# andrewmilson/sandstorm

Hardware: AMD Instinct MI355X
Metric: prove_wall_time_s (lower is better)
Workload: dtype u256 (Fp252, Montgomery R=2^256, 8 x u32 limbs)

## Files before the change

include/sandstorm_hip.h:

```cpp
#ifndef SANDSTORM_HIP_H
#define SANDSTORM_HIP_H
#include <stddef.h>
#include <stdint.h>

#ifdef __cplusplus
extern "C" {
#endif

typedef int ss_status;
enum {
    SS_OK = 0,
    SS_ERR_INVALID = 1,
    SS_ERR_HIP = 2,
    SS_ERR_NO_DEVICE = 3,
    SS_ERR_UNSUPPORTED = 4
};

typedef struct ss_ctx ss_ctx;

enum { SS_NTT_FORWARD = 0, SS_NTT_INVERSE = 1 };
enum { SS_ORDER_NATURAL = 0, SS_ORDER_BITREV = 1 };

enum {
    SS_HASH_KECCAK = 0,
// ... 20 lines not shown
void ss_ctx_destroy(ss_ctx *ctx);
ss_status ss_ctx_set_stream(ss_ctx *ctx, void *hip_stream);
ss_status ss_ctx_sync(ss_ctx *ctx);
ss_status ss_dev_alloc(ss_ctx *ctx, size_t bytes, void **d_out);
ss_status ss_dev_free(ss_ctx *ctx, void *d_ptr);
ss_status ss_ctx_trim(ss_ctx *ctx);
ss_status ss_upload(ss_ctx *ctx, void *d_dst, const void *src, size_t bytes);
ss_status ss_download(ss_ctx *ctx, void *dst, const void *d_src, size_t bytes);
ss_status ss_upload_async(ss_ctx *ctx, void *d_dst, const void *src, size_t bytes, uint64_t *ticket);
ss_status ss_wait_upload(ss_ctx *ctx, uint64_t ticket);
ss_status ss_dev_zero(ss_ctx *ctx, void *d_ptr, size_t bytes);

ss_status ss_dev_copy(ss_ctx *ctx, void *d_dst, const void *d_src, size_t bytes);
ss_status ss_dev_copy_2d(ss_ctx *ctx, void *d_dst, size_t dst_pitch, const void *d_src, size_t src_pitch, size_t width, size_t rows);
ss_status ss_bitrev_permute32(ss_ctx *ctx, const void *d_src, uint32_t log_n, void *d_dst);

typedef struct ss_comm ss_comm;
ss_status ss_comm_unique_id(uint8_t id_out[128]);
ss_status ss_comm_create(ss_ctx *ctx, const uint8_t id[128], uint32_t rank, uint32_t world, ss_comm **out);
void ss_comm_destroy(ss_comm *comm);
ss_status ss_comm_exchange(ss_comm *comm, uint32_t nsend, const uint32_t *send_peer, const void *const *d_send, const uint64_t *send_bytes,
                           uint32_t nrecv, const uint32_t *recv_peer, void *const *d_recv, const uint64_t *recv_bytes);
ss_status ss_comm_all_gather(ss_comm *comm, const void *d_send, uint64_t bytes, void *d_recv);

ss_status ss_ntt_fp252(ss_ctx *ctx, uint64_t *const *d_cols, uint32_t ncols, uint32_t log_n,
                       int direction, const uint64_t offset[4], int in_order, int out_order);

ss_status ss_lde_fp252(ss_ctx *ctx, const uint64_t *const *d_in, uint32_t ncols, uint32_t log_n,
                       uint32_t log_blowup, const uint64_t offset[4], uint64_t *const *d_evals,
                       uint64_t *const *d_coeffs);

ss_status ss_evaluate_fp252(ss_ctx *ctx, const uint64_t *const *d_coeffs, uint32_t ncols, uint32_t log_n,
                            uint32_t log_blowup, const uint64_t offset[4], uint64_t *const *d_evals);

ss_status ss_subsample_rows(ss_ctx *ctx, const uint64_t *const *d_in, uint32_t ncols, uint64_t nrows_out, uint32_t log_stride,
                            uint64_t *const *d_out);

enum { SS_NTT_PART_LOCAL = 0, SS_NTT_PART_CROSS = 1 };
ss_status ss_ntt_shard_fp252(ss_ctx *ctx, uint64_t *const *d_cols, uint32_t ncols, uint32_t log_n, uint32_t log_ranks,
                             uint32_t rank, int direction, const uint64_t offset[4], int part, uint32_t log_expand,
                             uint64_t *const *d_out);

ss_status ss_hash_rows(ss_ctx *ctx, int hash_kind, const uint64_t *const *d_cols, uint32_t ncols,
                       uint64_t nrows, uint8_t *d_digests);
ss_status ss_hash_rows_ex(ss_ctx *ctx, int hash_kind, const uint64_t *const *d_cols, uint32_t ncols,
                       uint64_t nrows, int row_order, uint8_t *d_digests);

ss_status ss_merkle_build(ss_ctx *ctx, int tree_kind, uint32_t n_friendly_layers, int leaf_kind,
                          const void *d_leaves, uint64_t n, uint8_t *d_nodes, uint8_t *d_tags,
                          uint8_t root_out[33]);
ss_status ss_merkle_build_ex(ss_ctx *ctx, int tree_kind, uint32_t n_friendly_layers, int leaf_kind,
                          const void *d_leaves, uint64_t n, int leaf_order, uint8_t *d_nodes, uint8_t *d_tags,
                          uint8_t root_out[33]);
ss_status ss_merkle_open(ss_ctx *ctx, const uint8_t *d_nodes, const uint8_t *d_tags, uint64_t n,
                         const uint64_t *idx, uint32_t nidx, uint8_t *out, uint8_t *out_tags);
ss_status ss_gather_rows(ss_ctx *ctx, const uint64_t *const *d_cols, uint32_t ncols,
                         const uint64_t *idx, uint32_t nidx, uint64_t *out );
typedef struct ss_gather_job {
    const void *const *d_cols;
    uint32_t ncols;
    uint32_t entry_bytes;
    const uint64_t *idx;
    uint32_t nidx;
    void *out;
} ss_gather_job;
ss_status ss_gather_batch(ss_ctx *ctx, const ss_gather_job *jobs, uint32_t njobs);
// ... 267 lines not shown
```

sandstorm_amd/_lib.py:

```python
import ctypes as C
import os
import sys

_HERE = os.path.dirname(os.path.abspath(__file__))
LIB_PATH = os.path.join(_HERE, "_build", "libsandstorm_hip.so")

HEADER_PATH = os.path.join(os.path.dirname(_HERE), "include", "sandstorm_hip.h")

SS_OK = 0


def header_abi_version():
    import re
    with open(HEADER_PATH) as f:
        m = re.search(r"#define\s+SS_ABI_VERSION\s+(\d+)u?", f.read())
    if not m:
        raise SandstormHipError("SS_ABI_VERSION not found in %s" % HEADER_PATH)
    return int(m.group(1))


class SandstormHipError(RuntimeError):
    pass


# ... 28 lines not shown

SIGNATURES = {
    "ss_last_error": (C.c_char_p, []),
    "ss_abi_version": (C.c_uint32, []),
    "ss_ctx_create": (C.c_int, [C.c_int, _vpp]),
    "ss_ctx_destroy": (None, [C.c_void_p]),
    "ss_ctx_set_stream": (C.c_int, [C.c_void_p, C.c_void_p]),
    "ss_ctx_sync": (C.c_int, [C.c_void_p]),
    "ss_dev_alloc": (C.c_int, [C.c_void_p, C.c_size_t, _vpp]),
    "ss_dev_free": (C.c_int, [C.c_void_p, C.c_void_p]),
    "ss_ctx_trim": (C.c_int, [C.c_void_p]),
    "ss_upload": (C.c_int, [C.c_void_p, C.c_void_p, C.c_void_p, C.c_size_t]),
    "ss_download": (C.c_int, [C.c_void_p, C.c_void_p, C.c_void_p, C.c_size_t]),
    "ss_dev_zero": (C.c_int, [C.c_void_p, C.c_void_p, C.c_size_t]),
    "ss_dev_copy": (C.c_int, [C.c_void_p, C.c_void_p, C.c_void_p, C.c_size_t]),
    "ss_dev_copy_2d": (C.c_int, [C.c_void_p, C.c_void_p, C.c_size_t, C.c_void_p, C.c_size_t, C.c_size_t, C.c_size_t]),
    "ss_bitrev_permute32": (C.c_int, [C.c_void_p, C.c_void_p, C.c_uint32, C.c_void_p]),
    "ss_comm_unique_id": (C.c_int, [C.c_char_p]),
    "ss_comm_create": (C.c_int, [C.c_void_p, C.c_char_p, C.c_uint32, C.c_uint32, _vpp]),
    "ss_comm_destroy": (None, [C.c_void_p]),
    "ss_comm_exchange": (C.c_int, [C.c_void_p, C.c_uint32, _u32p, _vpp, _u64p, C.c_uint32, _u32p, _vpp, _u64p]),
    "ss_comm_all_gather": (C.c_int, [C.c_void_p, C.c_void_p, C.c_uint64, C.c_void_p]),
    "ss_permutation_product": (C.c_int, [C.c_void_p, C.POINTER(PermOperand), C.POINTER(PermOperand), C.c_uint64, _u64p, _u64p,
                                         C.c_void_p, C.c_uint64, C.c_uint64, _u64p]),
    "ss_diluted_aggregate": (C.c_int, [C.c_void_p, C.c_void_p, C.c_uint64, C.c_uint64, C.c_uint64, _u64p, _u64p,
                                       C.c_void_p, C.c_uint64, C.c_uint64]),
    "ss_scale_strided": (C.c_int, [C.c_void_p, C.c_void_p, C.c_uint64, C.c_uint64, C.c_uint64, _u64p]),
    "ss_diluted_aggregate_block": (C.c_int, [C.c_void_p, C.c_void_p, C.c_uint64, C.c_uint64, C.c_uint64, C.c_int, _u64p, _u64p,
                                             C.c_void_p, _u64p]),
    "ss_affine_apply": (C.c_int, [C.c_void_p, C.c_void_p, C.c_uint64, _u64p, C.c_void_p, C.c_uint64, C.c_uint64]),
    "ss_ntt_fp252": (C.c_int, [C.c_void_p, _vpp, C.c_uint32, C.c_uint32, C.c_int, _u64p, C.c_int, C.c_int]),
    "ss_lde_fp252": (C.c_int, [C.c_void_p, _vpp, C.c_uint32, C.c_uint32, C.c_uint32, _u64p, _vpp, _vpp]),
    "ss_evaluate_fp252": (C.c_int, [C.c_void_p, _vpp, C.c_uint32, C.c_uint32, C.c_uint32, _u64p, _vpp]),
    "ss_subsample_rows": (C.c_int, [C.c_void_p, _vpp, C.c_uint32, C.c_uint64, C.c_uint32, _vpp]),
    "ss_ntt_shard_fp252": (C.c_int, [C.c_void_p, _vpp, C.c_uint32, C.c_uint32, C.c_uint32, C.c_uint32, C.c_int, _u64p, C.c_int, C.c_uint32, _vpp]),
    "ss_hash_rows": (C.c_int, [C.c_void_p, C.c_int, _vpp, C.c_uint32, C.c_uint64, C.c_void_p]),
    "ss_hash_rows_ex": (C.c_int, [C.c_void_p, C.c_int, _vpp, C.c_uint32, C.c_uint64, C.c_int, C.c_void_p]),
    "ss_merkle_build": (C.c_int, [C.c_void_p, C.c_int, C.c_uint32, C.c_int, C.c_void_p, C.c_uint64,
                                  C.c_void_p, C.c_void_p, _u8p]),
    "ss_merkle_build_ex": (C.c_int, [C.c_void_p, C.c_int, C.c_uint32, C.c_int, C.c_void_p, C.c_uint64, C.c_int,
                                  C.c_void_p, C.c_void_p, _u8p]),
    "ss_merkle_open": (C.c_int, [C.c_void_p, C.c_void_p, C.c_void_p, C.c_uint64, _u64p, C.c_uint32,
                                 C.c_void_p, C.c_void_p]),
    "ss_gather_rows": (C.c_int, [C.c_void_p, _vpp, C.c_uint32, _u64p, C.c_uint32, C.c_void_p]),
    "ss_gather_batch": (C.c_int, [C.c_void_p, C.POINTER(GatherJob), C.c_uint32]),
    "ss_trace_memory_image": (C.c_int, [C.c_void_p, C.c_void_p, C.c_uint64, C.c_void_p, C.c_uint64]),
    "ss_trace_cpu_cells": (C.c_int, [C.c_void_p, C.c_void_p, C.c_void_p, C.c_uint64, C.c_void_p, C.c_uint64, _u64p, C.c_uint64, C.c_void_p, C.c_void_p,
                                     C.c_void_p, C.c_void_p, C.c_void_p, C.c_void_p]),
    "ss_trace_builtin": (C.c_int, [C.c_void_p, _vpp, C.c_uint32, C.c_void_p, C.c_uint32, C.c_void_p, C.c_uint32, C.c_void_p, C.c_uint64, C.c_uint64,
                                   C.c_uint64, C.c_uint64, C.c_void_p]),
    "ss_trace_pedersen": (C.c_int, [C.c_void_p, _vpp, C.c_uint32, C.c_uint64, C.c_void_p, C.c_void_p, C.c_uint64, C.c_uint64, C.c_uint64, C.c_uint64, C.c_void_p,
                                    C.c_void_p]),
    "ss_trace_bitwise": (C.c_int, [C.c_void_p, _vpp, C.c_uint32, C.c_uint64, C.c_void_p, C.c_void_p, C.c_uint64, C.c_uint64, C.c_uint64, C.c_uint64, C.c_uint32,
                                   C.c_void_p, C.c_void_p]),
    "ss_trace_poseidon": (C.c_int, [C.c_void_p, _vpp, C.c_uint32, C.c_uint64, C.c_void_p, C.c_void_p, C.c_void_p, C.c_uint64, C.c_uint64, C.c_uint64, C.c_uint64,
                                    C.c_void_p, C.c_void_p]),
    "ss_trace_ec_op": (C.c_int, [C.c_void_p, _vpp, C.c_uint32, C.c_uint64, C.c_void_p, C.c_void_p, C.c_uint64, C.c_uint64, C.c_uint64, C.c_uint64, C.c_void_p,
                                 C.c_void_p]),
    "ss_trace_ecdsa": (C.c_int, [C.c_void_p, _vpp, C.c_uint32, C.c_uint64, C.c_void_p, C.c_void_p, C.c_void_p, C.c_uint64, C.c_uint64, C.c_uint64, C.c_uint64,
                                 C.c_void_p, C.c_void_p]),
    "ss_trace_rc_pool": (C.c_int, [C.c_void_p, C.c_void_p, C.c_void_p, C.c_void_p, C.c_uint64, C.c_void_p]),
    "ss_trace_rc_builtin": (C.c_int, [C.c_void_p, C.c_void_p, C.c_void_p, C.c_void_p, C.c_void_p, C.c_void_p, C.c_void_p]),
    "ss_trace_ordered_runs": (C.c_int, [C.c_void_p, C.c_void_p, C.c_uint64, C.c_uint64, C.c_uint64, C.c_void_p, C.c_uint32, C.c_uint32, C.c_int]),
    "ss_trace_patch": (C.c_int, [C.c_void_p, C.c_void_p, C.c_uint64, C.c_void_p, C.c_void_p, C.c_uint64]),
    "ss_trace_ordered_memory": (C.c_int, [C.c_void_p, C.c_uint64, C.c_void_p, C.c_void_p, C.c_void_p, C.c_void_p, C.c_void_p, C.c_uint32, C.c_uint64, _u64p,
                                          C.c_uint32, C.c_void_p]),
# ... 83 lines not shown
```

sandstorm_amd/csrc/capi.hip:

```cpp
#include <hip/hip_runtime.h>
#include <dlfcn.h>
#include <algorithm>
#include <cstdarg>
#include <chrono>
#include <cstdio>
#include <cstdlib>
#include <cstring>
#include <map>
#include <mutex>
#include <string>
#include <tuple>
#include <utility>
#include <vector>

#include "../../include/sandstorm_hip.h"
#include "fp252.h"
#include "fp252_host.h"
#include "kernels.h"
#include "quotient_gen.h"
#include "ext_scan.h"
#include "gl_ntt.h"

using namespace ss;

// ... 356 lines not shown
            s0 += r; rem -= r;
        }
    }
    return v;
}

ss_status run_forward(ss_ctx *ctx, const ColPtrs &cols, uint32_t ncols, uint32_t log_n, const Fp *tw,
                      uint32_t log_expand, bool canonical_out = true) {
    const uint32_t lt = (uint32_t)ntt_log_tile_max();
    const uint32_t log_tile = log_n < lt ? log_n : lt;
    std::vector<Pass> passes = plan_passes(log_n);
    if (log_expand >= log_n && log_n > 0) return fail(SS_ERR_INVALID, "log_blowup %u too large", log_expand);
    size_t start = 0;
    uint32_t skip = log_expand;
    while (start + 1 < passes.size() && skip >= passes[start].r) { skip -= passes[start].r; ++start; }
    if (skip >= passes[start].r && log_n > 0) return fail(SS_ERR_INVALID, "log_blowup %u too large", log_expand);
    ColPtrs inplace = cols;
    for (uint32_t c = 0; c < ncols; ++c) inplace.src[c] = cols.dst[c];
    for (size_t i = start; i < passes.size(); ++i) {
        const bool first = i == start;
        ss_ctx::Scope prof(ctx, SS_PROF_NTT_PASS);
        HIP_TRY(launch_ntt_pass(ctx->stream, NTT_MODE_DIT, first ? cols : inplace, ncols, tw, log_n, passes[i].s0,
                                passes[i].r, log_tile, first ? skip : 0, first ? log_expand : 0, 0, canonical_out && i + 1 == passes.size()));
    }
    return SS_OK;
}
ss_status get_inverse_plan(ss_ctx *ctx, uint32_t log_n, const Fp &offset, const Fp **tw, int *mode) {
    static const bool force_dif = getenv("SS_NTT_INVERSE_DIF") != nullptr;
    const bool cti = fp_eq(offset, fp_one()) && !force_dif;
    *mode = cti ? NTT_MODE_CTI : NTT_MODE_DIF;
    return ctx->get_plan(log_n, true, offset, tw, cti);
}
ss_status run_inverse(ss_ctx *ctx, const ColPtrs &cols, uint32_t ncols, uint32_t log_n, const Fp *tw, int mode,
                      uint32_t scale_log = ~0u, bool cti_trivial = true) {
    if (scale_log == ~0u) scale_log = log_n;
    const uint32_t lt = (uint32_t)ntt_log_tile_max();
    const uint32_t log_tile = log_n < lt ? log_n : lt;
    std::vector<Pass> passes = plan_passes(log_n);
    ColPtrs inplace = cols;
    for (uint32_t c = 0; c < ncols; ++c) inplace.src[c] = cols.dst[c];
    for (size_t i = passes.size(); i-- > 0;) {
        const bool first = i == passes.size() - 1;
        const bool last = i == 0;
        ss_ctx::Scope prof(ctx, SS_PROF_NTT_PASS);
        HIP_TRY(launch_ntt_pass(ctx->stream, mode, first ? cols : inplace, ncols, tw, log_n, passes[i].s0,
                                passes[i].r, log_tile, 0, 0, last ? scale_log : 0, last, cti_trivial));
    }
    return SS_OK;
}

bool valid_log(uint32_t log_n) { return log_n >= 1 && log_n <= 30; }

}

extern "C" {

const char *ss_last_error(void) { return g_err.c_str(); }
uint32_t ss_abi_version(void) { return SS_ABI_VERSION; }

ss_status ss_ctx_create(int device, ss_ctx **out) {
    if (!out) return fail(SS_ERR_INVALID, "out is NULL");
    int count = 0;
    hipError_t e = hipGetDeviceCount(&count);
    if (e != hipSuccess || count <= 0)
        return fail(SS_ERR_NO_DEVICE, "no HIP device: %s", e == hipSuccess ? "device count is 0" : hipGetErrorString(e));
    if (device < 0 || device >= count) return fail(SS_ERR_INVALID, "device %d out of range (%d)", device, count);
    HIP_TRY(hipSetDevice(device));
    hipDeviceProp_t prop;
    HIP_TRY(hipGetDeviceProperties(&prop, device));
    if (strncmp(prop.gcnArchName, "gfx950", 6) != 0)
        return fail(SS_ERR_NO_DEVICE, "device %d is %s; this library is built for gfx950 only", device, prop.gcnArchName);
    ss_ctx *ctx = new ss_ctx;
    ctx->device = device;
    HIP_TRY(hipStreamCreateWithFlags(&ctx->own_stream, hipStreamNonBlocking));
    ctx->stream = ctx->own_stream;
    HIP_TRY(hipMalloc(&ctx->d_small, 64 * sizeof(uint64_t)));
    HIP_TRY(ntt_set_func_attributes());
    HIP_TRY(gl_set_func_attributes());
    *out = ctx;
// ... 396 lines not shown
        ColPtrs inv, fwd;
        memset(&inv, 0, sizeof inv); memset(&fwd, 0, sizeof fwd);
        for (uint32_t c = 0; c < nc; ++c) {
            void *co = d_coeffs ? (void *)d_coeffs[base + c] : (void *)((char *)ctx->scratch + col_bytes * c);
            inv.src[c] = d_in[base + c]; inv.dst[c] = co;
            fwd.src[c] = co; fwd.dst[c] = d_evals[base + c];
        }
        st = run_inverse(ctx, inv, nc, log_n, tw_inv, inv_mode);
        if (st != SS_OK) return st;
        st = run_forward(ctx, fwd, nc, log_n + log_blowup, tw_fwd, log_blowup);
        if (st != SS_OK) return st;
    }
    return SS_OK;
}

ss_status ss_evaluate_fp252(ss_ctx *ctx, const uint64_t *const *d_coeffs, uint32_t ncols, uint32_t log_n,
                            uint32_t log_blowup, const uint64_t offset[4], uint64_t *const *d_evals) {
    if (!ctx || !d_coeffs || !d_evals) return fail(SS_ERR_INVALID, "NULL argument");
    if (!valid_log(log_n) || !valid_log(log_n + log_blowup)) return fail(SS_ERR_INVALID, "size out of range");
    if (has_null((const void *const *)d_coeffs, ncols) || has_null((const void *const *)d_evals, ncols)) return fail(SS_ERR_INVALID, "NULL column");
    const Fp off = offset ? fp_from_limbs64(offset) : fp_one();
    const Fp *tw = nullptr;
    ss_status st = ctx->get_plan(log_n + log_blowup, false, off, &tw);
    if (st != SS_OK) return st;
    for (uint32_t base = 0; base < ncols; base += MAX_COLS) {
        const uint32_t nc = ncols - base < (uint32_t)MAX_COLS ? ncols - base : (uint32_t)MAX_COLS;
        ColPtrs fwd;
        memset(&fwd, 0, sizeof fwd);
        for (uint32_t c = 0; c < nc; ++c) { fwd.src[c] = d_coeffs[base + c]; fwd.dst[c] = d_evals[base + c]; }
        st = run_forward(ctx, fwd, nc, log_n + log_blowup, tw, log_blowup);
        if (st != SS_OK) return st;
    }
    return SS_OK;
}

ss_status ss_subsample_rows(ss_ctx *ctx, const uint64_t *const *d_in, uint32_t ncols, uint64_t nrows_out, uint32_t log_stride,
                            uint64_t *const *d_out) {
    if (!ctx || !d_in || !d_out) return fail(SS_ERR_INVALID, "NULL argument");
    if (!ncols || !nrows_out) return fail(SS_ERR_INVALID, "no columns or no rows");
    if (log_stride > 4) return fail(SS_ERR_INVALID, "log_stride %u > 4", log_stride);
    if (nrows_out > (1ull << 40)) return fail(SS_ERR_INVALID, "size out of range");
    if (has_null((const void *const *)d_in, ncols) || has_null((const void *const *)d_out, ncols)) return fail(SS_ERR_INVALID, "NULL column");
    for (uint32_t base = 0; base < ncols; base += MAX_COLS) {
        const uint32_t nc = ncols - base < (uint32_t)MAX_COLS ? ncols - base : (uint32_t)MAX_COLS;
        ColPtrs cols;
        memset(&cols, 0, sizeof cols);
        for (uint32_t c = 0; c < nc; ++c) { cols.src[c] = d_in[base + c]; cols.dst[c] = d_out[base + c]; }
        HIP_TRY(launch_subsample_rows(ctx->stream, cols, nc, nrows_out, log_stride));
    }
    return SS_OK;
}

ss_status ss_ntt_shard_fp252(ss_ctx *ctx, uint64_t *const *d_cols, uint32_t ncols, uint32_t log_n, uint32_t log_ranks, uint32_t rank,
                             int direction, const uint64_t offset[4], int part, uint32_t log_expand, uint64_t *const *d_out) {
    if (!ctx || !d_cols) return fail(SS_ERR_INVALID, "NULL argument");
    if (direction != SS_NTT_FORWARD && direction != SS_NTT_INVERSE) return fail(SS_ERR_INVALID, "bad direction");
    if (part != SS_NTT_PART_LOCAL && part != SS_NTT_PART_CROSS) return fail(SS_ERR_INVALID, "bad part");
    if (!valid_log(log_n) || log_ranks == 0 || 2 * log_ranks > log_n || log_ranks > 7) return fail(SS_ERR_INVALID, "a transform of 2^%u points does not split over 2^%u ranks (needs n >= R^2)", log_n, log_ranks);
    if (rank >> log_ranks) return fail(SS_ERR_INVALID, "rank %u of %u", rank, 1u << log_ranks);
    if (ncols == 0) return fail(SS_ERR_INVALID, "no columns");
    if (has_null((const void *const *)d_cols, ncols) || (d_out && has_null((const void *const *)d_out, ncols))) return fail(SS_ERR_INVALID, "NULL column");
    for (uint32_t c0 = 0; ncols > (uint32_t)MAX_COLS && c0 < ncols; c0 += MAX_COLS) {
        const uint32_t k = ncols - c0 < (uint32_t)MAX_COLS ? ncols - c0 : (uint32_t)MAX_COLS;
        const ss_status st = ss_ntt_shard_fp252(ctx, d_cols + c0, k, log_n, log_ranks, rank, direction, offset, part, log_expand, d_out ? d_out + c0 : nullptr);
        if (st != SS_OK || c0 + k == ncols) return st;
    }
// ... 2185 lines not shown
```

sandstorm_amd/csrc/kernels.h:

```cpp
#pragma once
#include <hip/hip_runtime.h>
#include <stdint.h>
#include "fp252.h"

namespace ss {

static constexpr int MAX_COLS = 16;

struct ColPtrs {
    const void *src[MAX_COLS];
    void *dst[MAX_COLS];
};
struct ConstColPtrs {
    const void *p[MAX_COLS];
};

int ntt_log_tile_max();
static constexpr size_t NTT_PLAN_ENTRY_BYTES = 36;
enum { NTT_MODE_DIT = 0, NTT_MODE_DIF = 1, NTT_MODE_CTI = 2 };
struct NttWindow { uint32_t first, log_len; };
hipError_t launch_ntt_pass(hipStream_t st, int mode, const ColPtrs &cols, uint32_t ncols, const Fp *tw,
                           uint32_t log_n, uint32_t s0, uint32_t r, uint32_t log_tile, uint32_t u_first,
                           uint32_t log_expand, uint32_t scale_pow2, bool final_pass, bool cti_trivial = true,
                           const NttWindow *win = nullptr, uint64_t tw_entries = 0);
hipError_t launch_twiddles(hipStream_t st, Fp *tw, const Fp *pow_lo, const Fp *pow_hi, const Fp *hpow,
                           uint32_t log_n, bool h_is_one, bool bitrev_levels, const NttWindow *win = nullptr, uint32_t win_stages = 0);
static inline uint64_t ntt_window_plan_entries(const NttWindow &win, uint32_t stages) { return (((uint64_t)1 << stages) - 1ull) << win.log_len; }
hipError_t launch_bitrev(hipStream_t st, Fp *a, uint32_t log_n);
hipError_t launch_mul_bench(hipStream_t st, const Fp *a, const Fp *b, Fp *out, uint64_t n, uint32_t reps);
hipError_t ntt_set_func_attributes();

hipError_t launch_hash_rows(hipStream_t st, int kind, const ConstColPtrs &cols, uint32_t ncols,
                            uint64_t nrows, uint32_t brev_bits, uint8_t *digests);
hipError_t launch_bitrev_copy(hipStream_t st, const Fp *src, uint32_t log_n, Fp *dst);
hipError_t launch_hash_pairs(hipStream_t st, int kind, const uint8_t *in, uint64_t count, uint8_t *out);
hipError_t launch_hash_felt_pairs(hipStream_t st, int kind, const Fp *felts, uint64_t count, bool bitrev, uint8_t *out, uint8_t *leaves);
hipError_t launch_felts_to_be(hipStream_t st, const Fp *felts, uint64_t count, uint8_t *out);
hipError_t launch_pow_prefix(hipStream_t st, int coin_kind, const uint8_t digest[32], uint32_t bits,
                             uint64_t *d_prefix);
hipError_t launch_pow_grind(hipStream_t st, int coin_kind, const uint64_t *d_prefix, uint32_t bits,
                            uint64_t start, uint64_t count, unsigned long long *d_best);
hipError_t launch_gather32(hipStream_t st, const uint8_t *in, const uint64_t *d_idx, uint64_t n, uint8_t *out);
hipError_t launch_gather32_cols(hipStream_t st, const void *const *d_cols, uint32_t ncols, uint32_t c0, uint32_t row_cols, const uint64_t *d_idx,
                                uint64_t nidx, uint8_t *out);
hipError_t launch_gather8(hipStream_t st, const uint8_t *in, const uint64_t *d_idx, uint64_t n, uint8_t *out);

struct PedersenTables;
hipError_t pedersen_tables_create(hipStream_t st, PedersenTables **out);
void pedersen_tables_destroy(PedersenTables *t);
void pedersen_tables_trim();
static constexpr uint64_t PEDERSEN_TMP_FELTS_PER_HASH = 4;
hipError_t launch_pedersen_felts(hipStream_t st, const PedersenTables *t, const Fp *a, const Fp *b,
                                 uint64_t n, Fp *out, Fp *tmp);
hipError_t launch_pedersen_pairs(hipStream_t st, const PedersenTables *t, const uint8_t *in, uint64_t count,
                                 uint8_t *out, Fp *tmp);
hipError_t launch_pedersen_felt_pairs(hipStream_t st, const PedersenTables *t, const Fp *felts,
                                      uint64_t count, uint8_t *out, Fp *tmp);
// ... 212 lines not shown
```

sandstorm_amd/csrc/ntt.hip:

```cpp
#include <hip/hip_runtime.h>
#include <cstdlib>
#include "fp252.h"
#include "fl252.h"
#include "kernels.h"

#ifdef SS_NTT_ABL_NOBAR
#define NTT_SYNC() do {} while (0)
#else
#define NTT_SYNC() __syncthreads()
#endif
#ifndef SS_NTT_WAVE_PRIVATE
#define SS_NTT_WAVE_PRIVATE 1
#endif
#if defined(HIPEMU)
#define NTT_WAVE_SYNC() __syncthreads()
#elif defined(SS_NTT_ABL_NOBAR)
#define NTT_WAVE_SYNC() do {} while (0)
#else
#define NTT_WAVE_SYNC() do { __builtin_amdgcn_fence(__ATOMIC_RELEASE, "wavefront"); __builtin_amdgcn_wave_barrier(); \
                             __builtin_amdgcn_fence(__ATOMIC_ACQUIRE, "wavefront"); } while (0)
#endif

namespace ss {

// ... 107 lines not shown
    const uint4 *q = reinterpret_cast<const uint4 *>(p);
    uint4 a = q[0], b = q[1];
    Fp r;
    r.v[0] = a.x; r.v[1] = a.y; r.v[2] = a.z; r.v[3] = a.w;
    r.v[4] = b.x; r.v[5] = b.y; r.v[6] = b.z; r.v[7] = b.w;
    return r;
}
__device__ __forceinline__ void gstore(Fp *p, const Fp &x) {
#ifdef SS_NTT_ABL_NOGL
    if (!(x.v[0] == 0xdeadbeefu && x.v[3] == 77u)) return;
#endif
    uint4 *q = reinterpret_cast<uint4 *>(p);
    q[0] = make_uint4(x.v[0], x.v[1], x.v[2], x.v[3]);
    q[1] = make_uint4(x.v[4], x.v[5], x.v[6], x.v[7]);
}

struct PassParams {
    uint32_t log_n;
    uint32_t s0;
    uint32_t r;
    uint32_t log_tile;
    uint32_t u_first;
    uint32_t log_expand;
    uint32_t scale_pow2;
    uint32_t contig;
    uint32_t final_pass;
    uint32_t ncols;
    uint32_t xcd_map;
    uint32_t log_tiles;
    uint32_t tile0;
    uint32_t win_log1, win0;
    uint32_t cti_trivial;
    uint32_t tw_entries;
};
__device__ __forceinline__ uint32_t mem_index(const PassParams &p, uint32_t g) {
    if (!p.win_log1) return g;
    return ((g >> p.s0) << (p.win_log1 - 1u)) + ((g & ((1u << p.s0) - 1u)) - p.win0);
}

struct TwPlanes {
    const uint4 *lo, *hi;
    const u32 *top;
};
__device__ __forceinline__ Fl tw_load(const TwPlanes &tw, uint32_t idx) {
    const uint4 a4 = tw.lo[idx], b4 = tw.hi[idx];
    Fl t;
    t.l[0] = a4.x; t.l[1] = a4.y; t.l[2] = a4.z; t.l[3] = a4.w;
    t.l[4] = b4.x; t.l[5] = b4.y; t.l[6] = b4.z; t.l[7] = b4.w;
    t.l[8] = tw.top[idx];
    return t;
}

template <int MODE, int G, int ST>
__device__ __forceinline__ uint32_t stage_tw_index(const PassParams &p, uint32_t u, uint32_t g0, int pr) {
    constexpr int STC = ST < G ? ST : 0;
    const uint32_t gsh = p.s0 + u;
    const uint32_t s = gsh + STC;
    if (MODE == MODE_CTI) {
        const uint32_t level = p.log_n - 1u - s;
        return ((1u << level) - 1u) + ((g0 >> (gsh + G)) << (G - 1 - STC)) + (uint32_t)(pr >> STC);
    }
    const uint32_t klow = g0 & ((1u << gsh) - 1u);
    const int m = ((pr >> STC) << (STC + 1)) | (pr & ((1 << STC) - 1));
    if (p.win_log1)
        return ((((1u << (s - p.s0)) - 1u) + (klow >> p.s0)) << (p.win_log1 - 1u)) + ((klow & ((1u << p.s0) - 1u)) - p.win0)
               + ((uint32_t)(m & ((1 << STC) - 1)) << (u + p.win_log1 - 1u));
// ... 230 lines not shown
    if (MODE == MODE_DIT) {
        uint32_t u = p.u_first;
        bool first = true;
        while (u < p.r) {
            const uint32_t g = (p.r - u) >= (uint32_t)NTT_GMAX ? (uint32_t)NTT_GMAX : (p.r - u);
            const bool last = (u + g >= p.r);
            const bool fg = fuse && first, tg = fuse && last;
            if (fg) prev_private = group_private(u, g); else phase_sync(group_private(u, g));
            if (NTT_GMAX >= 3 && g == 3) radix_group<MODE, NTT_GMAX >= 3 ? 3 : 1>(t, tw, p, u, tile, false, fg, tg, src, dst);
            else if (g == 2) radix_group<MODE, 2>(t, tw, p, u, tile, false, fg, tg, src, dst);
            else radix_group<MODE, 1>(t, tw, p, u, tile, false, fg, tg, src, dst);
            u += g;
            first = false;
        }
    } else {
        uint32_t u = p.r;
        bool first = true;
        const bool top_pass = p.s0 + p.r == p.log_n;
        while (u > 0) {
            const uint32_t g = u >= (uint32_t)NTT_GMAX ? (uint32_t)NTT_GMAX : u;
            u -= g;
            const bool last = (u == 0);
            const bool fg = fuse && first, tg = fuse && last, top = top_pass && first;
            if (fg) prev_private = group_private(u, g); else phase_sync(group_private(u, g));
            if (NTT_GMAX >= 3 && g == 3) radix_group<MODE, NTT_GMAX >= 3 ? 3 : 1>(t, tw, p, u, tile, top, fg, tg, src, dst);
            else if (g == 2) radix_group<MODE, 2>(t, tw, p, u, tile, top, fg, tg, src, dst);
            else radix_group<MODE, 1>(t, tw, p, u, tile, top, fg, tg, src, dst);
            first = false;
        }
    }

    if (!fuse) {
        phase_sync(chunks);
        for (uint32_t x = x0; x < x_end; x += x_step)
            gstore(dst + mem_index(p, tile_gindex(p, tile, x)), pass_output<MODE>(p, lds_load(t, lds_addr<LG>(x)), false));
    }
}

__global__ void twiddle_kernel(Fp *__restrict__ tw, const Fp *__restrict__ pow_lo,
                               const Fp *__restrict__ pow_hi, const Fp *__restrict__ hpow,
                               uint32_t log_n, int h_is_one, int bitrev_levels, uint32_t win_s0, uint32_t win_log, uint32_t win0,
                               uint64_t total) {
    uint4 *plane_lo = reinterpret_cast<uint4 *>(tw), *plane_hi = plane_lo + total;
    u32 *plane_top = reinterpret_cast<u32 *>(plane_hi + total);
    for (uint64_t idx = blockIdx.x * (uint64_t)blockDim.x + threadIdx.x; idx < total;
         idx += (uint64_t)gridDim.x * blockDim.x) {
        uint32_t s = 63u - (uint32_t)__clzll(idx + 1ull);
        uint64_t k = idx + 1ull - (1ull << s);
        if (win_s0) {
            const uint64_t t = idx >> win_log;
            const uint32_t v = 63u - (uint32_t)__clzll(t + 1ull);
            s = win_s0 + v;
            k = ((t + 1ull - (1ull << v)) << win_s0) | (win0 + (idx & ((1ull << win_log) - 1ull)));
        }
        if (bitrev_levels && s) k = __brevll(k) >> (64u - s);
        const uint64_t e = k << (log_n - 1u - s);
        Fp t = fp_mul(gload(pow_lo + (e & 4095ull)), gload(pow_hi + (e >> 12)));
        if (!h_is_one) t = fp_mul(t, gload(hpow + s));
        const Fl l = fl_to_r280(t);
        plane_lo[idx] = make_uint4(l.l[0], l.l[1], l.l[2], l.l[3]);
        plane_hi[idx] = make_uint4(l.l[4], l.l[5], l.l[6], l.l[7]);
        plane_top[idx] = l.l[8];
    }
}

__global__ void bitrev_kernel(Fp *__restrict__ a, uint32_t log_n) {
    const uint64_t n = 1ull << log_n;
    for (uint64_t i = blockIdx.x * (uint64_t)blockDim.x + threadIdx.x; i < n;
         i += (uint64_t)gridDim.x * blockDim.x) {
        const uint64_t j = __brevll(i) >> (64u - log_n);
        if (i < j) {
            Fp x = gload(a + i), y = gload(a + j);
            gstore(a + i, y);
            gstore(a + j, x);
        }
    }
}

__global__ void mul_bench_kernel(const Fp *__restrict__ a, const Fp *__restrict__ b, Fp *__restrict__ out,
                                 uint64_t n, uint32_t reps) {
    for (uint64_t i = blockIdx.x * (uint64_t)blockDim.x + threadIdx.x; i < n;
         i += (uint64_t)gridDim.x * blockDim.x) {
        Fp x = gload(a + i);
        const Fp y = gload(b + i);
        for (uint32_t k = 0; k < reps; ++k) x = fp_mul(x, y);
        gstore(out + i, x);
    }
}

hipError_t launch_ntt_pass(hipStream_t st, int mode, const ColPtrs &cols, uint32_t ncols, const Fp *tw,
                           uint32_t log_n, uint32_t s0, uint32_t r, uint32_t log_tile, uint32_t u_first,
                           uint32_t log_expand, uint32_t scale_pow2, bool final_pass, bool cti_trivial, const NttWindow *win,
                           uint64_t tw_entries) {
    PassParams p;
    p.tw_entries = tw_entries ? (uint32_t)tw_entries : (uint32_t)((1ull << log_n) - 1ull);
    p.final_pass = final_pass ? 1u : 0u;
    p.log_n = log_n; p.s0 = s0; p.r = r; p.log_tile = log_tile; p.u_first = u_first;
    p.log_expand = log_expand; p.scale_pow2 = scale_pow2; p.contig = (s0 == 0);
    p.cti_trivial = cti_trivial ? 1u : 0u;
    p.log_tiles = log_n - log_tile; p.tile0 = 0; p.win_log1 = 0; p.win0 = 0;
    if (win) {
        const uint32_t log_t = log_tile - r;
        if (s0 + r != log_n || s0 == 0 || log_expand || win->log_len < log_t || (win->first & ((1u << win->log_len) - 1u))) return hipErrorInvalidValue;
        p.log_tiles = win->log_len - log_t;
        p.tile0 = win->first >> log_t;
        p.win_log1 = win->log_len + 1u;
        p.win0 = win->first;
    }
    const uint32_t tiles = 1u << p.log_tiles;
    static const bool no_xcd_map = getenv("SS_NTT_NO_XCD_MAP") != nullptr;
    p.ncols = ncols;
    p.xcd_map = (tiles >= 8 && ncols > 1 && !no_xcd_map) ? 1u : 0u;
    dim3 grid(tiles * ncols), block(mode == NTT_MODE_DIF ? SS_NTT_THREADS_DIF : SS_NTT_THREADS);
    if (mode == NTT_MODE_DIF) hipLaunchKernelGGL(ntt_pass_kernel<MODE_DIF>, grid, block, 0, st, cols, tw, p);
    else if (mode == NTT_MODE_CTI) hipLaunchKernelGGL(ntt_pass_kernel<MODE_CTI>, grid, block, 0, st, cols, tw, p);
    else hipLaunchKernelGGL(ntt_pass_kernel<MODE_DIT>, grid, block, 0, st, cols, tw, p);
    return hipGetLastError();
}

hipError_t launch_twiddles(hipStream_t st, Fp *tw, const Fp *pow_lo, const Fp *pow_hi, const Fp *hpow,
                           uint32_t log_n, bool h_is_one, bool bitrev_levels, const NttWindow *win, uint32_t win_stages) {
    const uint64_t total = win ? (((uint64_t)1 << win_stages) - 1ull) << win->log_len : (1ull << log_n) - 1ull;
    uint32_t blocks = (uint32_t)((total + 255) / 256);
    if (blocks > 4096) blocks = 4096;
    if (blocks == 0) blocks = 1;
    hipLaunchKernelGGL(twiddle_kernel, dim3(blocks), dim3(256), 0, st, tw, pow_lo, pow_hi, hpow, log_n,
                       h_is_one ? 1 : 0, bitrev_levels ? 1 : 0, win ? log_n - win_stages : 0u, win ? win->log_len : 0u, win ? win->first : 0u, total);
// ... 24 lines not shown
```

sandstorm_amd/host/prover.cpp:

```cpp
#include "prover.hpp"

#include <algorithm>
#include <chrono>
#include <cstdio>
#include <cstdlib>
#include <cstring>
#include <set>
#include <stdexcept>

namespace ssh {

static void ok(ss_status s) {
    if (s != SS_OK) throw std::runtime_error(ss_last_error());
}
static uint32_t log2u(uint64_t v) {
    uint32_t l = 0;
    while ((1ull << l) < v) ++l;
    if ((1ull << l) != v) throw std::runtime_error("not a power of two");
    return l;
}

uint32_t lde_log_blowup(const ProofOptions &opt) {
    const uint32_t f = opt.lde_blowup_factor;
    if (f != 2 && f != 4 && f != 8 && f != 16)
// ... 271 lines not shown
        ok(ss_lde_fp252(ctx_, (const uint64_t *const *)ext.cols.data(), ext.num_cols(), log_n, lb, g.data(), ext_lde.cols.data(),
                        ext_co.cols.data()));
        air.prepare_program(n, proof.challenges);
        mark("extension lde");
        ext_tree = commit(ext_lde);
        mark("extension commit");
        proof.has_extension = true;
        proof.extension_root = ext_tree->root();
        coin.reseed_with_digest(digest_of(proof.extension_root));
        lde_cols.insert(lde_cols.end(), ext_lde.cols.begin(), ext_lde.cols.end());
        coeff_cols.insert(coeff_cols.end(), ext_co.cols.begin(), ext_co.cols.end());
    }

    proof.composition_coeff = coin.draw();
    AirProgramData pd = air.build_program(n, proof.challenges, proof.composition_coeff);
    std::vector<uint64_t> consts = flat(pd.program.consts);
    ss_air_program prog;
    prog.code = pd.program.code.data(); prog.n_instr = pd.program.n_instr();
    prog.consts = consts.data(); prog.n_consts = (uint32_t)pd.program.consts.size();
    prog.d_tables = pd.d_tables; prog.table_desc = pd.table_desc.data(); prog.n_tables = (uint32_t)(pd.table_desc.size() / 2);
    prog.n_slots = pd.program.n_slots;
    mark("program build");
    DeviceBuffer comp_evals(ctx_, 32 * 2 * n);
    if (lb == 1) {
        ok(ss_eval_quotient(ctx_, &prog, (const uint64_t *const *)lde_cols.data(), (uint32_t)lde_cols.size(), log_n, 1, g.data(), comp_evals.u64()));
    } else {
        Matrix ce_cols = Matrix::alloc(ctx_, (uint32_t)lde_cols.size(), 2 * n);
        ok(ss_subsample_rows(ctx_, (const uint64_t *const *)lde_cols.data(), (uint32_t)lde_cols.size(), 2 * n, lb - 1, ce_cols.cols.data()));
        mark("subsample");
        ok(ss_eval_quotient(ctx_, &prog, (const uint64_t *const *)ce_cols.cols.data(), ce_cols.num_cols(), log_n, 1, g.data(), comp_evals.u64()));
    }
    mark("quotient");
    uint64_t *ce = comp_evals.u64();
    ok(ss_ntt_fp252(ctx_, &ce, 1, log_n + 1, SS_NTT_INVERSE, g.data(), SS_ORDER_NATURAL, SS_ORDER_BITREV));
    std::vector<uint64_t *> comp_coeffs;
    for (uint32_t k = 0; k < ncomp; ++k) comp_coeffs.push_back(ce + 4 * n * k);
    Matrix comp_lde = Matrix::alloc(ctx_, ncomp, N);
    ok(ss_evaluate_fp252(ctx_, (const uint64_t *const *)comp_coeffs.data(), ncomp, log_n, lb, g.data(), comp_lde.cols.data()));
    mark("composition lde");
    auto comp_tree = commit(comp_lde);
    mark("composition commit");
    proof.composition_root = comp_tree->root();
    coin.reseed_with_digest(digest_of(proof.composition_root));

    proof.z = coin.draw();
    std::vector<uint32_t> mask_col, mask_off;
    for (auto &c : air.mask) { mask_col.push_back(c.first); mask_off.push_back(c.second); }
    const uint32_t nmask = (uint32_t)air.mask.size();
    std::vector<uint64_t> ood_t(4 * nmask), ood_c(4 * ncomp);
    ok(ss_ood_eval(ctx_, (const uint64_t *const *)coeff_cols.data(), (uint32_t)coeff_cols.size(), log_n, mask_col.data(), mask_off.data(),
                   nmask, proof.z.data(), ood_t.data()));
    const Felt zc = felt_pow(proof.z, ncomp);
    ok(ss_poly_eval(ctx_, (const uint64_t *const *)comp_coeffs.data(), ncomp, log_n, zc.data(), ood_c.data()));
    for (uint32_t j = 0; j < nmask; ++j) { Felt f; memcpy(f.data(), ood_t.data() + 4 * j, 32); proof.ood_trace.push_back(f); }
    for (uint32_t k = 0; k < ncomp; ++k) { Felt f; memcpy(f.data(), ood_c.data() + 4 * k, 32); proof.ood_composition.push_back(f); }
    ok(ss_deep_prepare(ctx_, ncomp, log_n, g.data(), proof.z.data()));
    {
        std::vector<Felt> all = proof.ood_trace;
        all.insert(all.end(), proof.ood_composition.begin(), proof.ood_composition.end());
        coin.reseed_with_field_elements(all);
    }

    mark("ood");
    proof.deep_alpha = coin.draw();
    std::vector<Felt> coeffs;
    Felt cur = felt_from_u64(1);
    for (uint32_t i = 0; i < nmask + ncomp; ++i) { coeffs.push_back(cur); cur = felt_mul(cur, proof.deep_alpha); }
    std::vector<uint64_t> ct = flat(std::vector<Felt>(coeffs.begin(), coeffs.begin() + nmask));
    std::vector<uint64_t> cc = flat(std::vector<Felt>(coeffs.begin() + nmask, coeffs.end()));
    auto deep = std::make_shared<DeviceBuffer>(ctx_, 32 * N);
    ok(ss_deep_compose(ctx_, (const uint64_t *const *)lde_cols.data(), (uint32_t)lde_cols.size(), (const uint64_t *const *)comp_lde.cols.data(), ncomp,
                       log_n, lb, g.data(), mask_col.data(), mask_off.data(), nmask, ood_t.data(), ct.data(), ood_c.data(), cc.data(),
                       proof.z.data(), deep->u64()));

    mark("deep");
    std::vector<FriLayerState> layers = fri_commit_phase(ctx_, claim_, conv_, opt_, coin, proof, deep, log_N, n);

    mark("fri");
    proof.pow_nonce = proof_of_work(ctx_, claim_, coin, opt_, have_nonce_, nonce_);
    coin.reseed_with_int(proof.pow_nonce);
    proof.query_positions = coin.draw_queries(opt_.num_queries, N);
    const auto &pos = proof.query_positions;
    std::vector<uint64_t> nat = pos;
    if (conv_.bitrev_commit) for (auto &q : nat) q = brev(q, log_N);
    GatherBatch gb(ctx_);
// ... 121 lines not shown
```

Before: 0.2108.

## Fuse composition inverse NTT and coset LDE using plain-domain inverse with half scaling

Replaces the coset inverse NTT plus separate evaluate call for the composition polynomial with a new entry point. It runs a plain (non-coset) inverse NTT whose final pass scales the upper half by an offset-inverse factor, then a forward LDE on twiddles for the inverted offset. The OOD evaluation point is adjusted by g^-2 to match the changed coefficient basis. The aim is to drop the coset pre-scaling and reuse cached plain inverse plans, at the cost of extra algebraic bookkeeping and an env-var fallback path.

New measurement: 0.2102 (median of 4 runs). About the same (-0.3%).

```diff
diff --git a/include/sandstorm_hip.h b/include/sandstorm_hip.h
--- a/include/sandstorm_hip.h
+++ b/include/sandstorm_hip.h
@@ -76,6 +76,9 @@
 
 ss_status ss_evaluate_fp252(ss_ctx *ctx, const uint64_t *const *d_coeffs, uint32_t ncols, uint32_t log_n,
                             uint32_t log_blowup, const uint64_t offset[4], uint64_t *const *d_evals);
+
+ss_status ss_composition_lde_fp252(ss_ctx *ctx, uint64_t *d_evals, uint32_t log_n, uint32_t log_blowup, const uint64_t offset[4],
+                                   uint64_t *const *d_cols);
 
 ss_status ss_subsample_rows(ss_ctx *ctx, const uint64_t *const *d_in, uint32_t ncols, uint64_t nrows_out, uint32_t log_stride,
                             uint64_t *const *d_out);
diff --git a/sandstorm_amd/_lib.py b/sandstorm_amd/_lib.py
--- a/sandstorm_amd/_lib.py
+++ b/sandstorm_amd/_lib.py
@@ -84,6 +84,7 @@
     "ss_ntt_fp252": (C.c_int, [C.c_void_p, _vpp, C.c_uint32, C.c_uint32, C.c_int, _u64p, C.c_int, C.c_int]),
     "ss_lde_fp252": (C.c_int, [C.c_void_p, _vpp, C.c_uint32, C.c_uint32, C.c_uint32, _u64p, _vpp, _vpp]),
     "ss_evaluate_fp252": (C.c_int, [C.c_void_p, _vpp, C.c_uint32, C.c_uint32, C.c_uint32, _u64p, _vpp]),
+    "ss_composition_lde_fp252": (C.c_int, [C.c_void_p, C.c_void_p, C.c_uint32, C.c_uint32, _u64p, _vpp]),
     "ss_subsample_rows": (C.c_int, [C.c_void_p, _vpp, C.c_uint32, C.c_uint64, C.c_uint32, _vpp]),
     "ss_ntt_shard_fp252": (C.c_int, [C.c_void_p, _vpp, C.c_uint32, C.c_uint32, C.c_uint32, C.c_uint32, C.c_int, _u64p, C.c_int, C.c_uint32, _vpp]),
     "ss_hash_rows": (C.c_int, [C.c_void_p, C.c_int, _vpp, C.c_uint32, C.c_uint64, C.c_void_p]),
diff --git a/sandstorm_amd/csrc/capi.hip b/sandstorm_amd/csrc/capi.hip
--- a/sandstorm_amd/csrc/capi.hip
+++ b/sandstorm_amd/csrc/capi.hip
@@ -412,7 +412,7 @@
     return ctx->get_plan(log_n, true, offset, tw, cti);
 }
 ss_status run_inverse(ss_ctx *ctx, const ColPtrs &cols, uint32_t ncols, uint32_t log_n, const Fp *tw, int mode,
-                      uint32_t scale_log = ~0u, bool cti_trivial = true) {
+                      uint32_t scale_log = ~0u, bool cti_trivial = true, const NttHalfScale *half = nullptr) {
     if (scale_log == ~0u) scale_log = log_n;
     const uint32_t lt = (uint32_t)ntt_log_tile_max();
     const uint32_t log_tile = log_n < lt ? log_n : lt;
@@ -424,7 +424,7 @@
         const bool last = i == 0;
         ss_ctx::Scope prof(ctx, SS_PROF_NTT_PASS);
         HIP_TRY(launch_ntt_pass(ctx->stream, mode, first ? cols : inplace, ncols, tw, log_n, passes[i].s0,
-                                passes[i].r, log_tile, 0, 0, last ? scale_log : 0, last, cti_trivial));
+                                passes[i].r, log_tile, 0, 0, last ? scale_log : 0, last, cti_trivial, nullptr, 0, last ? half : nullptr));
     }
     return SS_OK;
 }
@@ -887,6 +887,39 @@
         if (st != SS_OK) return st;
     }
     return SS_OK;
+}
+
+ss_status ss_composition_lde_fp252(ss_ctx *ctx, uint64_t *d_evals, uint32_t log_n, uint32_t log_blowup, const uint64_t offset[4],
+                                   uint64_t *const *d_cols) {
+    if (!ctx || !d_evals || !d_cols || !offset) return fail(SS_ERR_INVALID, "NULL argument");
+    if (!valid_log(log_n) || !valid_log(log_n + 1) || log_blowup == 0 || !valid_log(log_n + log_blowup)) return fail(SS_ERR_INVALID, "size out of range");
+    if (has_null((const void *const *)d_cols, 2)) return fail(SS_ERR_INVALID, "NULL column");
+    const Fp off = fp_from_limbs64(offset);
+    if (fp_is_zero(off)) return fail(SS_ERR_INVALID, "offset is zero");
+    const Fp off_inv = fp_inv(off);
+    const Fp *tw_inv = nullptr, *tw_fwd = nullptr;
+    int inv_mode = NTT_MODE_DIF;
+    ss_status st = get_inverse_plan(ctx, log_n + 1, fp_one(), &tw_inv, &inv_mode);
+    if (st != SS_OK) return st;
+    st = ctx->get_plan(log_n + log_blowup, false, off_inv, &tw_fwd);
+    if (st != SS_OK) return st;
+    const uint64_t n = 1ull << log_n;
+    ColPtrs inv, fwd;
+    memset(&inv, 0, sizeof inv); memset(&fwd, 0, sizeof fwd);
+    inv.src[0] = d_evals; inv.dst[0] = d_evals;
+    for (uint32_t k = 0; k < 2; ++k) { fwd.src[k] = (Fp *)d_evals + n * k; fwd.dst[k] = d_cols[k]; }
+    if (inv_mode == NTT_MODE_CTI) {
+        NttHalfScale half;
+        half.from = (uint32_t)n;
+        half.c = fp_div_pow2(off_inv, log_n + 1);
+        st = run_inverse(ctx, inv, 1, log_n + 1, tw_inv, inv_mode, ~0u, true, &half);
+        if (st != SS_OK) return st;
+    } else {
+        st = run_inverse(ctx, inv, 1, log_n + 1, tw_inv, inv_mode);
+        if (st != SS_OK) return st;
+        HIP_TRY(launch_scale_strided(ctx->stream, (Fp *)d_evals + n, 1, 0, n, off_inv));
+    }
+    return run_forward(ctx, fwd, 2, log_n + log_blowup, tw_fwd, log_blowup);
 }
 
 ss_status ss_subsample_rows(ss_ctx *ctx, const uint64_t *const *d_in, uint32_t ncols, uint64_t nrows_out, uint32_t log_stride,
diff --git a/sandstorm_amd/csrc/kernels.h b/sandstorm_amd/csrc/kernels.h
--- a/sandstorm_amd/csrc/kernels.h
+++ b/sandstorm_amd/csrc/kernels.h
@@ -19,10 +19,12 @@
 static constexpr size_t NTT_PLAN_ENTRY_BYTES = 36;
 enum { NTT_MODE_DIT = 0, NTT_MODE_DIF = 1, NTT_MODE_CTI = 2 };
 struct NttWindow { uint32_t first, log_len; };
+struct NttHalfScale { uint32_t from; Fp c; };
 hipError_t launch_ntt_pass(hipStream_t st, int mode, const ColPtrs &cols, uint32_t ncols, const Fp *tw,
                            uint32_t log_n, uint32_t s0, uint32_t r, uint32_t log_tile, uint32_t u_first,
                            uint32_t log_expand, uint32_t scale_pow2, bool final_pass, bool cti_trivial = true,
-                           const NttWindow *win = nullptr, uint64_t tw_entries = 0);
+                           const NttWindow *win = nullptr, uint64_t tw_entries = 0,
+                           const NttHalfScale *half = nullptr);
 hipError_t launch_twiddles(hipStream_t st, Fp *tw, const Fp *pow_lo, const Fp *pow_hi, const Fp *hpow,
                            uint32_t log_n, bool h_is_one, bool bitrev_levels, const NttWindow *win = nullptr, uint32_t win_stages = 0);
 static inline uint64_t ntt_window_plan_entries(const NttWindow &win, uint32_t stages) { return (((uint64_t)1 << stages) - 1ull) << win.log_len; }
diff --git a/sandstorm_amd/csrc/ntt.hip b/sandstorm_amd/csrc/ntt.hip
--- a/sandstorm_amd/csrc/ntt.hip
+++ b/sandstorm_amd/csrc/ntt.hip
@@ -163,6 +163,8 @@
     uint32_t win_log1, win0;
     uint32_t cti_trivial;
     uint32_t tw_entries;
+    uint32_t half_on, half_from;
+    Fp half_c;
 };
 __device__ __forceinline__ uint32_t mem_index(const PassParams &p, uint32_t g) {
     if (!p.win_log1) return g;
@@ -459,6 +461,14 @@
 
     if (!fuse) {
         phase_sync(chunks);
+        if (MODE == MODE_CTI && p.half_on) {
+            for (uint32_t x = x0; x < x_end; x += x_step) {
+                const uint32_t gi = tile_gindex(p, tile, x);
+                const Fp v = fl_to_fp(lds_load(t, lds_addr<LG>(x)));
+                gstore(dst + gi, gi >= p.half_from ? fp_mul(v, p.half_c) : (p.scale_pow2 ? fp_div_pow2(v, p.scale_pow2) : v));
+            }
+            return;
+        }
         for (uint32_t x = x0; x < x_end; x += x_step)
             gstore(dst + mem_index(p, tile_gindex(p, tile, x)), pass_output<MODE>(p, lds_load(t, lds_addr<LG>(x)), false));
     }
@@ -518,8 +528,13 @@
 hipError_t launch_ntt_pass(hipStream_t st, int mode, const ColPtrs &cols, uint32_t ncols, const Fp *tw,
                            uint32_t log_n, uint32_t s0, uint32_t r, uint32_t log_tile, uint32_t u_first,
                            uint32_t log_expand, uint32_t scale_pow2, bool final_pass, bool cti_trivial, const NttWindow *win,
-                           uint64_t tw_entries) {
+                           uint64_t tw_entries, const NttHalfScale *half) {
     PassParams p;
+    p.half_on = 0; p.half_from = 0; p.half_c = fp_zero();
+    if (half) {
+        if (mode != NTT_MODE_CTI || !final_pass || s0 != 0 || win) return hipErrorInvalidValue;
+        p.half_on = 1u; p.half_from = half->from; p.half_c = half->c;
+    }
     p.tw_entries = tw_entries ? (uint32_t)tw_entries : (uint32_t)((1ull << log_n) - 1ull);
     p.final_pass = final_pass ? 1u : 0u;
     p.log_n = log_n; p.s0 = s0; p.r = r; p.log_tile = log_tile; p.u_first = u_first;
diff --git a/sandstorm_amd/host/prover.cpp b/sandstorm_amd/host/prover.cpp
--- a/sandstorm_amd/host/prover.cpp
+++ b/sandstorm_amd/host/prover.cpp
@@ -327,11 +327,16 @@
     }
     mark("quotient");
     uint64_t *ce = comp_evals.u64();
-    ok(ss_ntt_fp252(ctx_, &ce, 1, log_n + 1, SS_NTT_INVERSE, g.data(), SS_ORDER_NATURAL, SS_ORDER_BITREV));
     std::vector<uint64_t *> comp_coeffs;
     for (uint32_t k = 0; k < ncomp; ++k) comp_coeffs.push_back(ce + 4 * n * k);
     Matrix comp_lde = Matrix::alloc(ctx_, ncomp, N);
-    ok(ss_evaluate_fp252(ctx_, (const uint64_t *const *)comp_coeffs.data(), ncomp, log_n, lb, g.data(), comp_lde.cols.data()));
+    const bool coset_inverse = getenv("SS_COMPOSITION_COSET_INVERSE") != nullptr || getenv("SS_NTT_INVERSE_DIF") != nullptr;
+    if (coset_inverse) {
+        ok(ss_ntt_fp252(ctx_, &ce, 1, log_n + 1, SS_NTT_INVERSE, g.data(), SS_ORDER_NATURAL, SS_ORDER_BITREV));
+        ok(ss_evaluate_fp252(ctx_, (const uint64_t *const *)comp_coeffs.data(), ncomp, log_n, lb, g.data(), comp_lde.cols.data()));
+    } else {
+        ok(ss_composition_lde_fp252(ctx_, ce, log_n, lb, g.data(), comp_lde.cols.data()));
+    }
     mark("composition lde");
     auto comp_tree = commit(comp_lde);
     mark("composition commit");
@@ -345,7 +350,8 @@
     std::vector<uint64_t> ood_t(4 * nmask), ood_c(4 * ncomp);
     ok(ss_ood_eval(ctx_, (const uint64_t *const *)coeff_cols.data(), (uint32_t)coeff_cols.size(), log_n, mask_col.data(), mask_off.data(),
                    nmask, proof.z.data(), ood_t.data()));
-    const Felt zc = felt_pow(proof.z, ncomp);
+    Felt zc = felt_pow(proof.z, ncomp);
+    if (!coset_inverse) zc = felt_mul(zc, felt_inv(felt_mul(g, g)));
     ok(ss_poly_eval(ctx_, (const uint64_t *const *)comp_coeffs.data(), ncomp, log_n, zc.data(), ood_c.data()));
     for (uint32_t j = 0; j < nmask; ++j) { Felt f; memcpy(f.data(), ood_t.data() + 4 * j, 32); proof.ood_trace.push_back(f); }
     for (uint32_t k = 0; k < ncomp; ++k) { Felt f; memcpy(f.data(), ood_c.data() + 4 * k, 32); proof.ood_composition.push_back(f); }
```
